# a16z/jolt

Hardware: AMD Instinct MI355X
Metric: prover trace cycles/sec (sha3-shaped synthetic trace, sumcheck + HyperKZG hot path) (higher is better)
Workload: dtype u256 (BN254 Fr / Fq, 8x u32 Montgomery limbs; integer, bit-exact)

## Files before the change

include/jolt_hip.h:

```cpp
#ifndef JOLT_HIP_H
#define JOLT_HIP_H

#include <stddef.h>
#include <stdint.h>

#ifdef __cplusplus
extern "C" {
#endif

#define JOLT_HIP_ABI_VERSION 1

typedef struct { uint64_t l[4]; } jolt_fr_t;
typedef struct { uint64_t l[4]; } jolt_fq_t;
typedef struct { jolt_fq_t x, y, z; } jolt_g1_t;

typedef struct jolt_ctx jolt_ctx;
typedef struct jolt_table jolt_table;
typedef struct jolt_member jolt_member;
typedef struct jolt_srs jolt_srs;

enum {
    JOLT_OK = 0,
    JOLT_ERR_INVALID_ARG = 1,
    JOLT_ERR_NO_DEVICE = 2,
// ... 129 lines not shown

int32_t jolt_msm_g1(jolt_ctx *ctx, const jolt_srs *srs, const jolt_fr_t *scalars, size_t n, jolt_g1_t *out);
int32_t jolt_msm_g1_table(jolt_ctx *ctx, const jolt_srs *srs, const jolt_table *scalars, size_t n, jolt_g1_t *out);
int32_t jolt_msm_g1_table_full_width(jolt_ctx *ctx, const jolt_srs *srs, const jolt_table *scalars, size_t n, jolt_g1_t *out);
typedef struct jolt_msm_pending jolt_msm_pending;
int32_t jolt_msm_g1_tables_begin(jolt_ctx *ctx, const jolt_srs *srs, const jolt_table *const *scalars, const size_t *n, size_t count, jolt_msm_pending **out);
int32_t jolt_msm_g1_tables_finish(jolt_ctx *ctx, jolt_msm_pending *pending, jolt_g1_t *out);

int32_t jolt_hyperkzg_fold(jolt_ctx *ctx, const jolt_table *evals, const jolt_fr_t *point, size_t ell, jolt_table **levels_out);
int32_t jolt_hyperkzg_eval3(jolt_ctx *ctx, jolt_table *const *levels, size_t ell, const jolt_fr_t u[3], jolt_fr_t *v_out);
int32_t jolt_hyperkzg_rlc(jolt_ctx *ctx, jolt_table *const *levels, size_t ell, const jolt_fr_t *q, jolt_table **out);
int32_t jolt_hyperkzg_witness_poly(jolt_ctx *ctx, const jolt_table *f, const jolt_fr_t *u, jolt_table **out);

int32_t jolt_host_fr_mul(const jolt_fr_t *a, const jolt_fr_t *b, jolt_fr_t *out);
int32_t jolt_host_fr_add(const jolt_fr_t *a, const jolt_fr_t *b, jolt_fr_t *out);
int32_t jolt_host_fr_sub(const jolt_fr_t *a, const jolt_fr_t *b, jolt_fr_t *out);
int32_t jolt_host_fr_inv(const jolt_fr_t *a, jolt_fr_t *out);
int32_t jolt_host_fr_from_u64(uint64_t v, jolt_fr_t *out);
int32_t jolt_host_fr_mul_shifted(const jolt_fr_t *a, const jolt_fr_t *c, jolt_fr_t *out);
int32_t jolt_host_eq_evals(const jolt_fr_t *r, size_t n, const jolt_fr_t *scale, jolt_fr_t *out);
int32_t jolt_host_mul_limbs29(int32_t field, const jolt_fr_t *a, const jolt_fr_t *b, jolt_fr_t *out);
int32_t jolt_host_fq_limb_op(int32_t op, const jolt_fr_t *a, const jolt_fr_t *b, const jolt_fr_t *c, const jolt_fr_t *d, jolt_fr_t *out);
int32_t jolt_host_g1_sum_limb_form(const uint64_t *points, const uint8_t *negate, size_t count, jolt_g1_t *out);
int32_t jolt_host_fx_digits(const jolt_fr_t *scalar, uint32_t window_bits, uint32_t *keys_out, uint32_t *n_windows_out, uint32_t *buckets_out);
int32_t jolt_host_fx_segment_capacity(uint64_t n, uint32_t window_bits, uint32_t segment, uint32_t *capacity);
int32_t jolt_host_univariate_from_evals(const jolt_fr_t *evals, size_t n, jolt_fr_t *coeffs_out);
int32_t jolt_host_univariate_evaluate(const jolt_fr_t *coeffs, size_t n, const jolt_fr_t *x, jolt_fr_t *out);
int32_t jolt_host_gruen_poly_from_q(const jolt_fr_t *current_scalar, const jolt_fr_t *point_i, const jolt_fr_t *q_evals, size_t dq,
                                    const jolt_fr_t *s0_plus_s1, jolt_fr_t *coeffs_out);
int32_t jolt_host_gruen_poly_deg_3(const jolt_fr_t *current_scalar, const jolt_fr_t *point_i, const jolt_fr_t *q_constant,
                                   const jolt_fr_t *q_quadratic, const jolt_fr_t *s0_plus_s1, jolt_fr_t *coeffs_out);
int32_t jolt_host_booleanity_address_round(const jolt_fr_t *linear, const jolt_fr_t *squared, size_t n_polys, size_t stride, size_t len,
                                           const jolt_fr_t *weights, const jolt_fr_t *eq_address, jolt_fr_t *evals_out);
int32_t jolt_host_booleanity_address_bind(jolt_fr_t *linear, jolt_fr_t *squared, size_t n_polys, size_t stride, size_t len, jolt_fr_t *eq_address,
                                          const jolt_fr_t *challenge);
int32_t jolt_host_hamming_weights(const jolt_fr_t *gamma, const jolt_fr_t *r_address, const jolt_fr_t *virtualization_points, size_t n_polys, size_t log_k,
                                  jolt_fr_t *out);
int32_t jolt_host_pair_tables_round(const jolt_fr_t *g, const jolt_fr_t *w, size_t n_polys, size_t stride, size_t len, jolt_fr_t *evals_out );
int32_t jolt_host_pair_tables_bind(jolt_fr_t *g, jolt_fr_t *w, size_t n_polys, size_t stride, size_t len, const jolt_fr_t *challenge);
enum { JOLT_TRANSCRIPT_TEST = 0, JOLT_TRANSCRIPT_BLAKE2B_LEGACY = 1, JOLT_TRANSCRIPT_KECCAK_SPONGE = 2, JOLT_TRANSCRIPT_BLAKE2B_SPONGE = 3 };
#define JOLT_TRANSCRIPT_LABEL(kind, label) (((uint64_t)(kind) << 62) | ((uint64_t)(label) & (((uint64_t)1 << 62) - 1)))
typedef struct jolt_host_transcript jolt_host_transcript;
int32_t jolt_host_transcript_create(uint64_t label, jolt_host_transcript **out);
int32_t jolt_host_transcript_create_labelled(int32_t kind, const uint8_t *label, size_t label_len, jolt_host_transcript **out);
int32_t jolt_host_transcript_append_fr(jolt_host_transcript *t, const jolt_fr_t *values, size_t count);
int32_t jolt_host_transcript_append_bytes(jolt_host_transcript *t, const uint8_t *bytes, size_t count);
// ... 297 lines not shown
```

jolt_amd/csrc/fq_limb.hip.h:

```cpp
#pragma once
#include "field.hip.h"

namespace jolt {

struct FqL {
    uint32_t l[9];
};

namespace fql {
constexpr uint32_t P(int k) { return Limbs29<FqParams>::limb(k); }
constexpr uint32_t P2(int k) {
    uint64_t carry = 0, v = 0;
    for (int i = 0; i <= k; ++i) {
        v = 2ull * P(i) + carry;
        carry = v >> 29;
        v &= kMask29;
    }
    return (uint32_t)v;
}
constexpr uint32_t NINV = Limbs29<FqParams>::neg_inv();
constexpr uint32_t PM(int m, int k) {
    uint64_t carry = 0, v = 0;
    for (int i = 0; i <= k; ++i) {
        v = (uint64_t)m * P(i) + carry;
        carry = v >> 29;
        if (i < 8) v &= kMask29;
    }
    return (uint32_t)v;
}
}
#define JOLT_FQL_MP(m) {fql::PM(m, 0), fql::PM(m, 1), fql::PM(m, 2), fql::PM(m, 3), fql::PM(m, 4), fql::PM(m, 5), fql::PM(m, 6), fql::PM(m, 7), fql::PM(m, 8)}
#define JOLT_FQL_P {fql::P(0), fql::P(1), fql::P(2), fql::P(3), fql::P(4), fql::P(5), fql::P(6), fql::P(7), fql::P(8)}
#define JOLT_FQL_2P {fql::P2(0), fql::P2(1), fql::P2(2), fql::P2(3), fql::P2(4), fql::P2(5), fql::P2(6), fql::P2(7), fql::P2(8)}

JOLT_HD FqL fql_from_words(const Fq& a) {
    FqL r;
    to_limbs29<0>(a.l, r.l);
    return r;
}
JOLT_HD FqL fql_zero() {
    FqL r;
#pragma unroll
    for (int k = 0; k < 9; ++k) r.l[k] = 0;
    return r;
}
JOLT_HD bool fql_is_zero(const FqL& a) {
    constexpr uint32_t PL[9] = JOLT_FQL_P;
    uint32_t any = 0, diff = 0;
#pragma unroll
    for (int k = 0; k < 9; ++k) {
        any |= a.l[k];
        diff |= a.l[k] ^ PL[k];
    }
    return any == 0 || diff == 0;
}
JOLT_HD FqL fql_add(const FqL& a, const FqL& b) {
    constexpr uint32_t P2L[9] = JOLT_FQL_2P;
// ... 29 lines not shown
    }
    uint32_t carry = 0;
#pragma unroll
    for (int k = 0; k < 9; ++k) {
        const uint32_t t = d[k] + P2L[k] + carry;
        e[k] = t & kMask29;
        carry = t >> 29;
    }
    FqL r;
#pragma unroll
    for (int k = 0; k < 9; ++k) r.l[k] = borrow ? e[k] : d[k];
    return r;
}
JOLT_HD FqL fql_dbl(const FqL& a) { return fql_add(a, a); }

JOLT_HD FqL fql_mul(const FqL& a, const FqL& b) {
    constexpr uint32_t PL[9] = JOLT_FQL_P;
    uint32_t M[9];
    FqL r;
    uint64_t acc = 0;
#pragma unroll
    for (int k = 0; k < 9; ++k) {
#pragma unroll
        for (int i = 0; i <= k; ++i) acc += (uint64_t)a.l[i] * b.l[k - i];
#pragma unroll
        for (int i = 0; i < k; ++i) acc += (uint64_t)M[i] * PL[k - i];
        M[k] = ((uint32_t)acc * fql::NINV) & kMask29;
        acc += (uint64_t)M[k] * PL[0];
        acc >>= 29;
    }
#pragma unroll
    for (int k = 9; k < 18; ++k) {
#pragma unroll
        for (int i = k - 8; i < 9; ++i) acc += (uint64_t)a.l[i] * b.l[k - i];
#pragma unroll
        for (int i = k - 8; i < 9; ++i) acc += (uint64_t)M[i] * PL[k - i];
        r.l[k - 9] = (uint32_t)acc & kMask29;
        acc >>= 29;
    }
    return r;
}
JOLT_HD FqL fql_mul2(const FqL& a, const FqL& b, const FqL& c, const FqL& d) {
    constexpr uint32_t PL[9] = JOLT_FQL_P;
    uint32_t M[9];
    FqL r;
    uint64_t acc = 0;
#pragma unroll
    for (int k = 0; k < 9; ++k) {
#pragma unroll
        for (int i = 0; i <= k; ++i) {
            acc += (uint64_t)a.l[i] * b.l[k - i];
            acc += (uint64_t)c.l[i] * d.l[k - i];
        }
#pragma unroll
        for (int i = 0; i < k; ++i) acc += (uint64_t)M[i] * PL[k - i];
        M[k] = ((uint32_t)acc * fql::NINV) & kMask29;
        acc += (uint64_t)M[k] * PL[0];
        acc >>= 29;
    }
#pragma unroll
    for (int k = 9; k < 18; ++k) {
#pragma unroll
        for (int i = k - 8; i < 9; ++i) {
            acc += (uint64_t)a.l[i] * b.l[k - i];
            acc += (uint64_t)c.l[i] * d.l[k - i];
        }
#pragma unroll
        for (int i = k - 8; i < 9; ++i) acc += (uint64_t)M[i] * PL[k - i];
        r.l[k - 9] = (uint32_t)acc & kMask29;
        acc >>= 29;
    }
    return r;
}
JOLT_HD FqL fql_sqr(const FqL& a) {
    constexpr uint32_t PL[9] = JOLT_FQL_P;
    uint32_t M[9], a2[9];
#pragma unroll
    for (int k = 0; k < 9; ++k) a2[k] = a.l[k] << 1;
    FqL r;
    uint64_t acc = 0;
#pragma unroll
    for (int k = 0; k < 9; ++k) {
#pragma unroll
        for (int i = 0; 2 * i < k; ++i) acc += (uint64_t)a.l[i] * a2[k - i];
        if (k % 2 == 0) acc += (uint64_t)a.l[k / 2] * a.l[k / 2];
#pragma unroll
        for (int i = 0; i < k; ++i) acc += (uint64_t)M[i] * PL[k - i];
        M[k] = ((uint32_t)acc * fql::NINV) & kMask29;
        acc += (uint64_t)M[k] * PL[0];
        acc >>= 29;
    }
#pragma unroll
    for (int k = 9; k < 18; ++k) {
#pragma unroll
        for (int i = k - 8; 2 * i < k; ++i) acc += (uint64_t)a.l[i] * a2[k - i];
        if (k % 2 == 0) acc += (uint64_t)a.l[k / 2] * a.l[k / 2];
#pragma unroll
        for (int i = k - 8; i < 9; ++i) acc += (uint64_t)M[i] * PL[k - i];
        r.l[k - 9] = (uint32_t)acc & kMask29;
        acc >>= 29;
    }
    return r;
}
JOLT_HD Fq fql_to_std(const FqL& a, const FqL& r256) {
    const FqL v = fql_mul(a, r256);
    Fq out;
#pragma unroll
    for (int j = 0; j < 8; ++j) {
        const int k = (32 * j) / 29, s = 32 * j - 29 * k;
        uint32_t w = v.l[k] >> s;
        w |= v.l[k + 1] << (29 - s);
        if (58 - s < 32 && k + 2 < 9) w |= v.l[k + 2] << (58 - s);
        out.l[j] = w;
    }
    return reduce_once(out, 0u);
}

template <int M, bool WITH_C>
JOLT_HD FqL fql_diff(const FqL& a, const FqL& b, const FqL& c) {
    constexpr uint32_t MP[9] = JOLT_FQL_MP(M);
    FqL r;
    int32_t carry = 0;
#pragma unroll
    for (int k = 0; k < 9; ++k) {
        int32_t t = (int32_t)a.l[k] + (int32_t)MP[k] - (int32_t)b.l[k] + carry;
        if (WITH_C) t -= (int32_t)(c.l[k] << 1);
        r.l[k] = k < 8 ? ((uint32_t)t & kMask29) : (uint32_t)t;
        carry = t >> 29;
    }
    return r;
}
template <int MAX>
JOLT_HD bool fql_is_multiple_of_p(const FqL& a) {
    bool hit = false;
#pragma unroll
    for (int m = 1; m <= MAX; ++m) {
        uint32_t diff = 0;
#pragma unroll
        for (int k = 0; k < 9; ++k) diff |= a.l[k] ^ fql::PM(m, k);
        hit = hit || diff == 0;
    }
    return hit;
}

struct G1XyzzL {
    FqL x, y, zz, zzz;
};
JOLT_HD G1XyzzL g1xl_identity() {
    G1XyzzL r;
// ... 26 lines not shown
        r.zz = one;
        r.zzz = one;
        return r;
    }
    const FqL U2 = fql_mul(qx, p.zz);
    const FqL S2 = fql_mul(qy, p.zzz);
    const FqL P = fql_diff<8, false>(U2, p.x, U2);
    const FqL R = fql_diff<4, false>(S2, p.y, S2);
    const FqL PP = fql_sqr(P);
    const FqL PPP = fql_mul(P, PP);
    const FqL Q = fql_mul(p.x, PP);
    G1XyzzL r;
    r.zz = fql_mul(p.zz, PP);
    if (fql_is_zero(r.zz)) {
        if (fql_is_multiple_of_p<5>(R)) return g1xl_double_affine(qx, qy);
        return g1xl_identity();
    }
    r.x = fql_diff<6, true>(fql_sqr(R), PPP, Q);
    r.y = fql_mul2(R, fql_diff<8, false>(Q, r.x, Q), fql_diff<4, false>(fql_zero(), p.y, Q), PPP);
    r.zzz = fql_mul(p.zzz, PPP);
    return r;
}

}
```

jolt_amd/csrc/host_mirror.hip:

```cpp
#include "host_mirror.hpp"

#include <algorithm>
#include <array>
#include <string>

#include "member.hpp"

using namespace jolt;

namespace jolt_host {

Fr fr_mul_pow_2(Fr a, size_t k) {
    for (size_t i = 0; i < k; ++i) a = add(a, a);
    return a;
}
void fr_to_bytes_le(const Fr& a, uint8_t out[32]) {
    Fr c = from_mont(a);
    for (int i = 0; i < 8; ++i)
        for (int j = 0; j < 4; ++j) out[4 * i + j] = (uint8_t)(c.l[i] >> (8 * j));
}
Fr fr_from_challenge_bytes(const uint8_t* b, size_t n) {
    uint8_t buf[16] = {0};
    std::memcpy(buf, b, n < 16 ? n : 16);
    Fr r = Fr::zero();
// ... 710 lines not shown
    };
    const FqL r256 = fql_from_words(Fq::one());
    FqL r;
    switch (op) {
        case 0: r = fql_mul(load(a), load(b)); break;
        case 1: r = fql_sqr(load(a)); break;
        case 2: r = fql_mul2(load(a), load(b), load(c), load(d)); break;
        case 3: r = fql_mul(fql_diff<8, false>(load(a), load(b), load(a)), load(c)); break;
        case 4: r = fql_mul(fql_diff<6, true>(load(a), load(b), load(c)), load(d)); break;
        default: return JOLT_ERR_INVALID_ARG;
    }
    const Fq res = fql_to_std(r, r256);
    std::memcpy(out, &res, sizeof(res));
    return JOLT_OK;
}
extern "C" int32_t jolt_host_g1_sum_limb_form(const uint64_t* points , const uint8_t* negate, size_t count, jolt_g1_t* out) {
    if ((!points && count) || !out) return JOLT_ERR_INVALID_ARG;
    using namespace jolt;
    Fq thirty_two = Fq::zero();
    thirty_two.l[0] = 32;
    const Fq m32 = to_mont(thirty_two);
    const FqL one = fql_from_words(m32), r256 = fql_from_words(Fq::one());
    G1XyzzL acc = g1xl_identity();
    for (size_t i = 0; i < count; ++i) {
        G1Affine p;
        std::memcpy(&p, points + 8 * i, sizeof(p));
        if (g1_aff_is_inf(p)) continue;
        if (negate && negate[i]) p.y = neg(p.y);
        acc = g1xl_add_mixed(acc, fql_from_words(mul(p.x, m32)), fql_from_words(mul(p.y, m32)), one);
    }
    G1Jac r = g1_identity();
    if (!g1xl_is_identity(acc)) {
        r.x = fql_to_std(fql_mul(acc.x, fql_sqr(acc.zz)), r256);
        r.y = fql_to_std(fql_mul(acc.y, fql_sqr(acc.zzz)), r256);
        r.z = fql_to_std(acc.zzz, r256);
    }
    std::memcpy(out, &r, sizeof(r));
    return JOLT_OK;
}
extern "C" int32_t jolt_host_fr_add(const jolt_fr_t* a, const jolt_fr_t* b, jolt_fr_t* out) {
    if (!a || !b || !out) return JOLT_ERR_INVALID_ARG;
    fr_to_abi(out, add(fr_from_abi(a), fr_from_abi(b)));
    return JOLT_OK;
}
extern "C" int32_t jolt_host_fr_sub(const jolt_fr_t* a, const jolt_fr_t* b, jolt_fr_t* out) {
    if (!a || !b || !out) return JOLT_ERR_INVALID_ARG;
    fr_to_abi(out, sub(fr_from_abi(a), fr_from_abi(b)));
    return JOLT_OK;
}
extern "C" int32_t jolt_host_fr_inv(const jolt_fr_t* a, jolt_fr_t* out) {
    if (!a || !out) return JOLT_ERR_INVALID_ARG;
    Fr v = fr_from_abi(a);
    if (v.is_zero()) return JOLT_ERR_NOT_INVERTIBLE;
    fr_to_abi(out, inv(v));
    return JOLT_OK;
}
extern "C" int32_t jolt_host_fr_from_u64(uint64_t v, jolt_fr_t* out) {
    if (!out) return JOLT_ERR_INVALID_ARG;
    fr_to_abi(out, fr_from_u64(v));
    return JOLT_OK;
// ... 300 lines not shown
```

jolt_amd/csrc/msm_kernels.hip.h:

```cpp
#pragma once
#include "g1.hip.h"
#include "fq_limb.hip.h"
#include "poly_kernels.hip.h"

#ifndef JOLT_BUCKET_WAVES
#define JOLT_BUCKET_WAVES 3
#endif
namespace jolt {
namespace msmk {
namespace {

#ifndef JOLT_BUCKET_XYZZ
#define JOLT_BUCKET_XYZZ 1
#endif
constexpr int kLaneCap = 128;
constexpr int kHeavySeg = 1024;
constexpr int kPeelMax = 16;

__device__ __forceinline__ G1Affine ld_aff(const G1Affine* p) {
    const uint4* q = reinterpret_cast<const uint4*>(p);
    uint4 a = q[0], b = q[1], c = q[2], d = q[3];
    G1Affine r;
    r.x.l[0] = a.x; r.x.l[1] = a.y; r.x.l[2] = a.z; r.x.l[3] = a.w; r.x.l[4] = b.x; r.x.l[5] = b.y; r.x.l[6] = b.z; r.x.l[7] = b.w;
    r.y.l[0] = c.x; r.y.l[1] = c.y; r.y.l[2] = c.z; r.y.l[3] = c.w; r.y.l[4] = d.x; r.y.l[5] = d.y; r.y.l[6] = d.z; r.y.l[7] = d.w;
// ... 197 lines not shown
            if (more) {
                vn = src[kn];
                pn = ld_aff(bases + (vn & 0x7FFFFFFFu));
            }
            if (v >> 31) p.y = neg(p.y);
            acc = JOLT_BUCKET_ADD(acc, p);
            if (!more) break;
            v = vn;
            p = pn;
            k = kn;
        }
        return JOLT_BUCKET_OUT(acc);
    }
#undef JOLT_BUCKET_ADD
#undef JOLT_BUCKET_OUT
}

struct LformConsts {
    Fq one_l;
    Fq r256;
};
__device__ __forceinline__ G1Jac sum_bucket_points_lform(const uint32_t* __restrict__ src, const G1Affine* __restrict__ bases, uint32_t lo, uint32_t hi, uint32_t stride,
                                                         const LformConsts& lc) {
    G1XyzzL acc = g1xl_identity();
    if (lo >= hi) return g1_identity();
    const FqL one = fql_from_words(lc.one_l);
    uint32_t v = src[lo];
    G1Affine p = ld_aff(bases + (v & 0x7FFFFFFFu));
    for (uint32_t k = lo;;) {
        const uint32_t kn = k + stride;
        const bool more = kn < hi;
        uint32_t vn = 0;
        G1Affine pn = p;
        if (more) {
            vn = src[kn];
            pn = ld_aff(bases + (vn & 0x7FFFFFFFu));
        }
        if (!g1_aff_is_inf(p)) {
            if (v >> 31) p.y = neg(p.y);
            acc = g1xl_add_mixed(acc, fql_from_words(p.x), fql_from_words(p.y), one);
        }
        if (!more) break;
        v = vn;
        p = pn;
        k = kn;
    }
    if (g1xl_is_identity(acc)) return g1_identity();
    const FqL r256 = fql_from_words(lc.r256);
    G1Jac out;
    out.x = fql_to_std(fql_mul(acc.x, fql_sqr(acc.zz)), r256);
    out.y = fql_to_std(fql_mul(acc.y, fql_sqr(acc.zzz)), r256);
    out.z = fql_to_std(acc.zzz, r256);
    return out;
}

template <int CH>
__device__ __forceinline__ void stage_indices(uint32_t* __restrict__ col, const uint32_t* __restrict__ src, uint32_t first, uint32_t cnt) {
#pragma unroll 1
    for (int j0 = 0; j0 < CH; j0 += 8) {
        uint32_t t[8];
#pragma unroll
        for (int j = 0; j < 8; ++j) t[j] = first + j0 + j < cnt ? src[first + j0 + j] : 0u;
#pragma unroll
        for (int j = 0; j < 8; ++j) col[(j0 + j) * kBlock] = t[j];
        if (first + j0 + 8 >= cnt) break;
    }
}
template <int CH>
__device__ __forceinline__ G1Jac sum_bucket_points_lform_staged(const uint32_t* __restrict__ src, const G1Affine* __restrict__ bases, uint32_t cnt, const LformConsts& lc,
                                                                uint32_t* __restrict__ col ) {
    if (cnt == 0) return g1_identity();
    G1XyzzL acc = g1xl_identity();
    const FqL one = fql_from_words(lc.one_l);
    stage_indices<CH>(col, src, 0u, cnt);
    uint32_t v = col[0], first = 0;
    G1Affine p = ld_aff(bases + (v & 0x7FFFFFFFu));
    for (uint32_t k = 0;;) {
        const uint32_t kn = k + 1;
        const bool more = kn < cnt;
        uint32_t vn = 0;
        G1Affine pn = p;
        if (more) {
            if (kn - first == (uint32_t)CH) {
                first = kn;
                stage_indices<CH>(col, src, first, cnt);
            }
            vn = col[(kn - first) * kBlock];
            pn = ld_aff(bases + (vn & 0x7FFFFFFFu));
        }
        if (!g1_aff_is_inf(p)) {
            if (v >> 31) p.y = neg(p.y);
            acc = g1xl_add_mixed(acc, fql_from_words(p.x), fql_from_words(p.y), one);
        }
        if (!more) break;
        v = vn;
        p = pn;
        k = kn;
    }
    if (g1xl_is_identity(acc)) return g1_identity();
    const FqL r256 = fql_from_words(lc.r256);
    G1Jac out;
    out.x = fql_to_std(fql_mul(acc.x, fql_sqr(acc.zz)), r256);
    out.y = fql_to_std(fql_mul(acc.y, fql_sqr(acc.zzz)), r256);
    out.z = fql_to_std(acc.zzz, r256);
    return out;
}

template <bool PIPELINED>
__global__ __launch_bounds__(kBlock) __attribute__((amdgpu_waves_per_eu(JOLT_BUCKET_WAVES, JOLT_BUCKET_WAVES))) void k_msm_buckets_light(const uint32_t* __restrict__ hist, const uint32_t* __restrict__ offsets,
                                                             const uint32_t* __restrict__ sorted, const G1Affine* __restrict__ bases, size_t n,
                                                             uint32_t B, int L, uint32_t heavy_threshold, G1Jac* __restrict__ buckets,
                                                             size_t n_windows) {
    uint32_t gt = blockIdx.x * kBlock + threadIdx.x;
    uint32_t b = gt / L + 1, sub = gt % L;
    const size_t wi = (size_t)blockIdx.z * gridDim.y + blockIdx.y;
    if (wi >= n_windows) return;
    const size_t w = n_windows - 1 - wi;
    bool mine = b <= B;
    size_t slot = (size_t)w * (B + 1) + (mine ? b : 0);
    uint32_t cnt = mine ? hist[slot] : 0;
    if (cnt > heavy_threshold) { cnt = 0; mine = false; }
    G1Jac acc = sum_bucket_points<PIPELINED>(sorted + (size_t)w * n + offsets[slot], bases, sub, cnt, (uint32_t)L);
// ... 75 lines not shown
```

jolt_amd/csrc/pcs.hip:

```cpp
#include <algorithm>
#include <cstdlib>
#include <cstring>

#include "grid_hint.hpp"
#include "ints.hpp"
#include "msm_kernels.hip.h"
#include "onehot.hpp"
#include "srs.hpp"
#include "term_map.hip.h"

using namespace jolt;
using namespace jolt::msmk;

int32_t jolt_internal_table_new(jolt_ctx* ctx, size_t len, jolt_table** out);
extern "C" int32_t jolt_grid_commit_onehot_range(jolt_ctx* ctx, const jolt_srs* srs, const jolt_onehot* source, size_t cycle_lo, size_t cycle_hi, jolt_g1_t* out);

namespace {

constexpr int kGridSumBlocks = 512;

template <bool LFORM>
__global__ __launch_bounds__(kBlock) __attribute__((amdgpu_waves_per_eu(JOLT_BUCKET_WAVES, JOLT_BUCKET_WAVES))) void k_grid_onehot_sum(
    const uint8_t* __restrict__ idx, uint32_t wide, size_t grid_cycles, size_t lo, size_t cycles, const G1Affine* __restrict__ bases, G1Jac* __restrict__ partial,
    LformConsts lc, uint32_t shift) {
    const size_t p = blockIdx.y, cls = blockIdx.z;
    const uint8_t* col = hot_col(idx, p * grid_cycles, wide);
    const size_t stride = ((size_t)gridDim.x * kBlock) << shift, folded_cycles = grid_cycles >> shift;
    G1Xyzz acc = g1x_identity();
    G1XyzzL acc_l = g1xl_identity();
    const FqL one = fql_from_words(lc.one_l);
    size_t j = lo + cls + (((size_t)blockIdx.x * kBlock + threadIdx.x) << shift);
    uint32_t a = j < cycles ? hot_load(col, j, wide) : kColdIdx;
    G1Affine pt;
    pt.x = Fq::zero();
    pt.y = Fq::zero();
    if (a != kColdIdx) pt = ld_aff(bases + (size_t)a * folded_cycles + (j >> shift));
    while (j < cycles) {
        const size_t jn = j + stride;
        const uint32_t an = jn < cycles ? hot_load(col, jn, wide) : kColdIdx;
        G1Affine pn;
        pn.x = Fq::zero();
        pn.y = Fq::zero();
        if (an != kColdIdx) pn = ld_aff(bases + (size_t)an * folded_cycles + (jn >> shift));
        if (LFORM) {
            if (!g1_aff_is_inf(pt)) acc_l = g1xl_add_mixed(acc_l, fql_from_words(pt.x), fql_from_words(pt.y), one);
        } else {
            acc = g1x_add_mixed(acc, pt);
        }
        pt = pn;
        j = jn;
    }
    G1Jac mine = g1x_to_jac(acc);
    if (LFORM) {
        mine = g1_identity();
        if (!g1xl_is_identity(acc_l)) {
            const FqL r256 = fql_from_words(lc.r256);
            mine.x = fql_to_std(fql_mul(acc_l.x, fql_sqr(acc_l.zz)), r256);
            mine.y = fql_to_std(fql_mul(acc_l.y, fql_sqr(acc_l.zzz)), r256);
            mine.z = fql_to_std(acc_l.zzz, r256);
        }
    }
    const G1Jac total = wave_sum_g1(mine, 64);
    if ((threadIdx.x & 63) == 0) partial[((cls * gridDim.y + p) * gridDim.x + blockIdx.x) * (kBlock / 64) + (threadIdx.x >> 6)] = total;
}
__global__ __launch_bounds__(64) void k_grid_onehot_fold(const G1Jac* __restrict__ partial, uint32_t count, G1Jac* __restrict__ out, uint32_t n_cols, uint32_t out_cols,
                                                         uint32_t first) {
    const size_t p = blockIdx.x;
    G1Jac acc = g1_identity();
    for (uint32_t k = threadIdx.x; k < count; k += 64) acc = g1_add(acc, partial[p * count + k]);
    acc = wave_sum_g1(acc, 64);
    if (threadIdx.x == 0) out[(p / n_cols) * out_cols + first + (p % n_cols)] = acc;
}
__global__ __launch_bounds__(1024) void k_grid_hint_combine(const G1Jac* __restrict__ points, const Fr* __restrict__ scalars, const uint32_t* __restrict__ offsets,
                                                            G1Jac* __restrict__ out) {
    __shared__ G1Jac wave_total[16];
    const uint32_t lo = offsets[blockIdx.x], hi = offsets[blockIdx.x + 1];
    G1Jac acc = g1_identity();
    for (uint32_t i = lo + threadIdx.x; i < hi; i += blockDim.x) {
// ... 425 lines not shown
```

jolt_amd/ffi.py:

```python
import ctypes as C
import os

import numpy as np

_HERE = os.path.dirname(os.path.abspath(__file__))
LIB_PATH = os.path.join(_HERE, "libjolt_hip.so")

STATUS = {0: "ok", 1: "invalid argument", 2: "no device", 3: "oom", 4: "hip error", 5: "size mismatch", 6: "unsupported",
          7: "not fully bound", 8: "round check failed", 9: "srs too small", 10: "empty point", 11: "not invertible"}
ORDER_LOW_TO_HIGH, ORDER_HIGH_TO_LOW = 0, 1
MEMBER_FLAG_SKIP_ONE = 1
MEMBER_FLAG_BORROW_TABLES = 2


class JoltError(RuntimeError):
    def __init__(self, status, where, detail=""):
        self.status = status
        super().__init__(f"{where}: status {status} ({STATUS.get(status, '?')}) {detail}")


class MemberDesc(C.Structure):
    _fields_ = [("n_tables", C.c_uint32), ("n_terms", C.c_uint32), ("degree", C.c_uint32), ("order", C.c_int32),
                ("term_offsets", C.c_void_p), ("factors", C.c_void_p), ("coeffs", C.c_void_p)]

# ... 1595 lines not shown
        if self.h:
            lib().jolt_read_raf_destroy(self.ctx.h, self.h)
            self.h = None


Context.read_raf = lambda self, lookup_index, table_index, raf_flag, n_tables: ReadRaf(self, lookup_index, table_index, raf_flag, n_tables)


def host_fq_limb_op(op, a, b=None, c=None, d=None):
    o = fr_array(1)
    arg = lambda x: _p(fr(x)) if x is not None else None
    _ck(lib().jolt_host_fq_limb_op(C.c_int32(op), arg(a), arg(b), arg(c), arg(d), _p(o)), "jolt_host_fq_limb_op")
    return o[0]


def host_g1_sum_limb_form(points, negate=None):
    pts = np.ascontiguousarray(points, dtype=np.uint64).reshape(-1, 8)
    neg = np.ascontiguousarray(negate if negate is not None else np.zeros(pts.shape[0]), dtype=np.uint8)
    out = g1_array(1)
    _ck(lib().jolt_host_g1_sum_limb_form(pts.ctypes.data_as(C.c_void_p), neg.ctypes.data_as(C.c_void_p), C.c_size_t(pts.shape[0]), _p(out)), "jolt_host_g1_sum_limb_form")
    return out[0]


def host_fx_digits(scalar, window_bits):
    keys = np.zeros(64, dtype=np.uint32)
    nw, nb = C.c_uint32(), C.c_uint32()
    _ck(lib().jolt_host_fx_digits(_p(fr(scalar)), C.c_uint32(window_bits), keys.ctypes.data_as(C.c_void_p), C.byref(nw), C.byref(nb)), "jolt_host_fx_digits")
    return [(-1 if int(k) >> 31 else 1) * (int(k) & 0x7FFFFFFF) for k in keys[: nw.value]], nb.value


def host_fx_segment_capacity(n, window_bits, segment):
    cap = C.c_uint32()
    _ck(lib().jolt_host_fx_segment_capacity(C.c_uint64(n), C.c_uint32(window_bits), C.c_uint32(segment), C.byref(cap)), "jolt_host_fx_segment_capacity")
    return int(cap.value)


def host_suffix_mle(kind, bits, length):
    out = C.c_uint64()
    _ck(lib().jolt_host_suffix_mle(C.c_uint32(kind), C.c_uint64(bits & (2**64 - 1)), C.c_uint64((bits >> 64) & (2**64 - 1)), C.c_uint32(length), C.byref(out)), "jolt_host_suffix_mle")
    return out.value


def host_small_scalar_dot(values, scalars):
    v = fr(values).reshape(-1, 4)
    sc = np.array([[int(x) & (2**64 - 1), (int(x) >> 64) & (2**64 - 1)] for x in scalars], dtype=np.uint64).reshape(-1, 2)
    o = fr_array(1)
# ... 342 lines not shown
```

rust/jolt-kernels-hip/src/ffi.rs:

```rust
#![allow(non_camel_case_types, clippy::too_many_arguments, clippy::missing_safety_doc)]
use core::ffi::{c_char, c_void};

pub const JOLT_HIP_ABI_VERSION: i32 = 1;

#[repr(C)]
#[derive(Clone, Copy, Debug, Default, PartialEq, Eq)]
pub struct jolt_fr_t {
    pub l: [u64; 4],
}
#[repr(C)]
#[derive(Clone, Copy, Debug, Default, PartialEq, Eq)]
pub struct jolt_fq_t {
    pub l: [u64; 4],
}
#[repr(C)]
#[derive(Clone, Copy, Debug, Default, PartialEq, Eq)]
pub struct jolt_g1_t {
    pub x: jolt_fq_t,
    pub y: jolt_fq_t,
    pub z: jolt_fq_t,
}
#[repr(C)]
pub struct jolt_ctx {
    _private: [u8; 0],
// ... 197 lines not shown
    pub fn jolt_srs_precompute_windows(ctx: *mut jolt_ctx, srs: *mut jolt_srs, window_bits: u32, min_terms: usize) -> i32;
    pub fn jolt_msm_profile_buckets(ctx: *mut jolt_ctx, enable: i32) -> i32;
    pub fn jolt_msm_profile_buckets_last(ctx: *mut jolt_ctx, ms: *mut f32, additions: *mut u64) -> i32;
    pub fn jolt_ctx_measure_mad_peak(ctx: *mut jolt_ctx, target_ms: f32, mads_per_s: *mut f64, timed_ms: *mut f32, launches: *mut u32) -> i32;
    pub fn jolt_msm_g1(ctx: *mut jolt_ctx, srs: *const jolt_srs, scalars: *const jolt_fr_t, n: usize, out: *mut jolt_g1_t) -> i32;
    pub fn jolt_msm_g1_table(ctx: *mut jolt_ctx, srs: *const jolt_srs, scalars: *const jolt_table, n: usize, out: *mut jolt_g1_t) -> i32;
    pub fn jolt_msm_g1_table_full_width(ctx: *mut jolt_ctx, srs: *const jolt_srs, scalars: *const jolt_table, n: usize, out: *mut jolt_g1_t) -> i32;
    pub fn jolt_msm_g1_tables_begin(ctx: *mut jolt_ctx, srs: *const jolt_srs, scalars: *const *const jolt_table, n: *const usize, count: usize, out: *mut *mut jolt_msm_pending) -> i32;
    pub fn jolt_msm_g1_tables_finish(ctx: *mut jolt_ctx, pending: *mut jolt_msm_pending, out: *mut jolt_g1_t) -> i32;
    pub fn jolt_hyperkzg_fold(ctx: *mut jolt_ctx, evals: *const jolt_table, point: *const jolt_fr_t, ell: usize, levels_out: *mut *mut jolt_table) -> i32;
    pub fn jolt_hyperkzg_eval3(ctx: *mut jolt_ctx, levels: *const *mut jolt_table, ell: usize, u: *const jolt_fr_t, v_out: *mut jolt_fr_t) -> i32;
    pub fn jolt_hyperkzg_rlc(ctx: *mut jolt_ctx, levels: *const *mut jolt_table, ell: usize, q: *const jolt_fr_t, out: *mut *mut jolt_table) -> i32;
    pub fn jolt_hyperkzg_witness_poly(ctx: *mut jolt_ctx, f: *const jolt_table, u: *const jolt_fr_t, out: *mut *mut jolt_table) -> i32;
    pub fn jolt_host_fr_mul(a: *const jolt_fr_t, b: *const jolt_fr_t, out: *mut jolt_fr_t) -> i32;
    pub fn jolt_host_fr_add(a: *const jolt_fr_t, b: *const jolt_fr_t, out: *mut jolt_fr_t) -> i32;
    pub fn jolt_host_fr_sub(a: *const jolt_fr_t, b: *const jolt_fr_t, out: *mut jolt_fr_t) -> i32;
    pub fn jolt_host_fr_inv(a: *const jolt_fr_t, out: *mut jolt_fr_t) -> i32;
    pub fn jolt_host_fr_from_u64(v: u64, out: *mut jolt_fr_t) -> i32;
    pub fn jolt_host_fr_mul_shifted(a: *const jolt_fr_t, c: *const jolt_fr_t, out: *mut jolt_fr_t) -> i32;
    pub fn jolt_host_eq_evals(r: *const jolt_fr_t, n: usize, scale: *const jolt_fr_t, out: *mut jolt_fr_t) -> i32;
    pub fn jolt_host_mul_limbs29(field: i32, a: *const jolt_fr_t, b: *const jolt_fr_t, out: *mut jolt_fr_t) -> i32;
    pub fn jolt_host_fq_limb_op(op: i32, a: *const jolt_fr_t, b: *const jolt_fr_t, c: *const jolt_fr_t, d: *const jolt_fr_t, out: *mut jolt_fr_t) -> i32;
    pub fn jolt_host_g1_sum_limb_form(points: *const u64, negate: *const u8, count: usize, out: *mut jolt_g1_t) -> i32;
    pub fn jolt_host_fx_digits(scalar: *const jolt_fr_t, window_bits: u32, keys_out: *mut u32, n_windows_out: *mut u32, buckets_out: *mut u32) -> i32;
    pub fn jolt_host_fx_segment_capacity(n: u64, window_bits: u32, segment: u32, capacity: *mut u32) -> i32;
    pub fn jolt_host_univariate_from_evals(evals: *const jolt_fr_t, n: usize, coeffs_out: *mut jolt_fr_t) -> i32;
    pub fn jolt_host_univariate_evaluate(coeffs: *const jolt_fr_t, n: usize, x: *const jolt_fr_t, out: *mut jolt_fr_t) -> i32;
    pub fn jolt_host_gruen_poly_from_q(current_scalar: *const jolt_fr_t, point_i: *const jolt_fr_t, q_evals: *const jolt_fr_t, dq: usize, s0_plus_s1: *const jolt_fr_t, coeffs_out: *mut jolt_fr_t) -> i32;
    pub fn jolt_host_gruen_poly_deg_3(current_scalar: *const jolt_fr_t, point_i: *const jolt_fr_t, q_constant: *const jolt_fr_t, q_quadratic: *const jolt_fr_t, s0_plus_s1: *const jolt_fr_t, coeffs_out: *mut jolt_fr_t) -> i32;
    pub fn jolt_host_booleanity_address_round(linear: *const jolt_fr_t, squared: *const jolt_fr_t, n_polys: usize, stride: usize, len: usize, weights: *const jolt_fr_t, eq_address: *const jolt_fr_t, evals_out: *mut jolt_fr_t) -> i32;
    pub fn jolt_host_booleanity_address_bind(linear: *mut jolt_fr_t, squared: *mut jolt_fr_t, n_polys: usize, stride: usize, len: usize, eq_address: *mut jolt_fr_t, challenge: *const jolt_fr_t) -> i32;
    pub fn jolt_host_hamming_weights(gamma: *const jolt_fr_t, r_address: *const jolt_fr_t, virtualization_points: *const jolt_fr_t, n_polys: usize, log_k: usize, out: *mut jolt_fr_t) -> i32;
    pub fn jolt_host_pair_tables_round(g: *const jolt_fr_t, w: *const jolt_fr_t, n_polys: usize, stride: usize, len: usize, evals_out: *mut jolt_fr_t) -> i32;
    pub fn jolt_host_pair_tables_bind(g: *mut jolt_fr_t, w: *mut jolt_fr_t, n_polys: usize, stride: usize, len: usize, challenge: *const jolt_fr_t) -> i32;
    pub fn jolt_host_transcript_create(label: u64, out: *mut *mut jolt_host_transcript) -> i32;
    pub fn jolt_host_transcript_create_labelled(kind: i32, label: *const u8, label_len: usize, out: *mut *mut jolt_host_transcript) -> i32;
    pub fn jolt_host_transcript_append_fr(t: *mut jolt_host_transcript, values: *const jolt_fr_t, count: usize) -> i32;
    pub fn jolt_host_transcript_append_bytes(t: *mut jolt_host_transcript, bytes: *const u8, count: usize) -> i32;
    pub fn jolt_host_transcript_append_label(t: *mut jolt_host_transcript, label: *const c_char, with_count: i32, count: u64) -> i32;
    pub fn jolt_host_transcript_append_u64_word(t: *mut jolt_host_transcript, value: u64) -> i32;
    pub fn jolt_host_transcript_append_round_poly(t: *mut jolt_host_transcript, label: *const c_char, coefficients: *const jolt_fr_t, count: usize) -> i32;
    pub fn jolt_host_transcript_challenge(t: *mut jolt_host_transcript, full_width: i32, out: *mut jolt_fr_t) -> i32;
    pub fn jolt_host_transcript_state(t: *const jolt_host_transcript, out32: *mut u8) -> i32;
    pub fn jolt_host_transcript_destroy(t: *mut jolt_host_transcript) -> i32;
    pub fn jolt_host_blake2b(r#in: *const u8, n: usize, outlen: usize, out: *mut u8) -> i32;
    pub fn jolt_host_keccak_f1600(state200: *mut u8) -> i32;
// ... 167 lines not shown
```

Baseline: 11.37 million.

## Split mixed G1 add into branch-free common path with wave-uniform rare fallback

Restructures the limb-form XYZZ mixed addition used in MSM bucket sums and the PCS accumulation. Each loop now seeds the accumulator from the first point, runs a branch-free common addition with a signed-difference trick that folds y-negation into R, and takes the identity/doubling fallback only when a wave-wide vote flags a suspect result, reloading the point from memory in that case. The field mul/sqr inner products are also rewritten to use inline v_mad_u64_u32 accumulate chains with scalar-register constants. The aim is to cut per-add divergence and branch overhead and to shorten the multiply chains. The risk is in correctness of the suspect detection (it checks only limb 0), and in the compiler scheduling the asm chains less well. A host test mirror is added.

```diff
diff --git a/include/jolt_hip.h b/include/jolt_hip.h
--- a/include/jolt_hip.h
+++ b/include/jolt_hip.h
@@ -175,6 +175,7 @@
 int32_t jolt_host_mul_limbs29(int32_t field, const jolt_fr_t *a, const jolt_fr_t *b, jolt_fr_t *out);
 int32_t jolt_host_fq_limb_op(int32_t op, const jolt_fr_t *a, const jolt_fr_t *b, const jolt_fr_t *c, const jolt_fr_t *d, jolt_fr_t *out);
 int32_t jolt_host_g1_sum_limb_form(const uint64_t *points, const uint8_t *negate, size_t count, jolt_g1_t *out);
+int32_t jolt_host_g1xl_add_paths(const uint32_t *acc, const uint32_t *q, int32_t negate, uint32_t *common, uint32_t *full, uint32_t *step, int32_t *suspect, uint32_t *canon);
 int32_t jolt_host_fx_digits(const jolt_fr_t *scalar, uint32_t window_bits, uint32_t *keys_out, uint32_t *n_windows_out, uint32_t *buckets_out);
 int32_t jolt_host_fx_segment_capacity(uint64_t n, uint32_t window_bits, uint32_t segment, uint32_t *capacity);
 int32_t jolt_host_univariate_from_evals(const jolt_fr_t *evals, size_t n, jolt_fr_t *coeffs_out);
diff --git a/jolt_amd/csrc/fq_limb.hip.h b/jolt_amd/csrc/fq_limb.hip.h
--- a/jolt_amd/csrc/fq_limb.hip.h
+++ b/jolt_amd/csrc/fq_limb.hip.h
@@ -1,5 +1,6 @@
 #pragma once
 #include "field.hip.h"
+#include "g1.hip.h"
 
 namespace jolt {
 
@@ -28,11 +29,39 @@
     }
     return (uint32_t)v;
 }
+constexpr uint32_t PM1(int m, int k) {
+    uint64_t carry = 0, v = 0;
+    for (int i = 0; i <= k; ++i) {
+        v = (uint64_t)m * P(i) + 1 + carry;
+        carry = v >> 29;
+        if (i < 8) v &= kMask29;
+    }
+    return (uint32_t)v;
+}
+constexpr uint32_t PM1H(int m, int k) { return (PM1(m, k) >> 1) | (k < 8 ? (PM1(m, k + 1) & 1u) << 28 : 0u); }
+static_assert((PM1(3, 0) & 1u) == 0 && (PM1(11, 0) & 1u) == 0, "m p + ones must be even");
 }
 #define JOLT_FQL_MP(m) {fql::PM(m, 0), fql::PM(m, 1), fql::PM(m, 2), fql::PM(m, 3), fql::PM(m, 4), fql::PM(m, 5), fql::PM(m, 6), fql::PM(m, 7), fql::PM(m, 8)}
 #define JOLT_FQL_P {fql::P(0), fql::P(1), fql::P(2), fql::P(3), fql::P(4), fql::P(5), fql::P(6), fql::P(7), fql::P(8)}
 #define JOLT_FQL_2P {fql::P2(0), fql::P2(1), fql::P2(2), fql::P2(3), fql::P2(4), fql::P2(5), fql::P2(6), fql::P2(7), fql::P2(8)}
 
+#ifndef JOLT_FQL_ONE_CHAIN
+#define JOLT_FQL_ONE_CHAIN 1
+#endif
+JOLT_HD void fql_mac(uint64_t& acc, uint32_t a, uint32_t b) {
+#if defined(__HIP_DEVICE_COMPILE__) && JOLT_FQL_ONE_CHAIN
+    asm("v_mad_u64_u32 %0, vcc, %1, %2, %0" : "+v"(acc) : "v"(a), "v"(b) : "vcc");
+#else
+    acc += (uint64_t)a * b;
+#endif
+}
+JOLT_HD void fql_mac_const(uint64_t& acc, uint32_t a, uint32_t c) {
+#if defined(__HIP_DEVICE_COMPILE__) && JOLT_FQL_ONE_CHAIN
+    asm("v_mad_u64_u32 %0, vcc, %1, %2, %0" : "+v"(acc) : "v"(a), "s"(c) : "vcc");
+#else
+    acc += (uint64_t)a * c;
+#endif
+}
 JOLT_HD FqL fql_from_words(const Fq& a) {
     FqL r;
     to_limbs29<0>(a.l, r.l);
@@ -108,19 +137,19 @@
 #pragma unroll
     for (int k = 0; k < 9; ++k) {
 #pragma unroll
-        for (int i = 0; i <= k; ++i) acc += (uint64_t)a.l[i] * b.l[k - i];
-#pragma unroll
-        for (int i = 0; i < k; ++i) acc += (uint64_t)M[i] * PL[k - i];
+        for (int i = 0; i <= k; ++i) fql_mac(acc, a.l[i], b.l[k - i]);
+#pragma unroll
+        for (int i = 0; i < k; ++i) fql_mac_const(acc, M[i], PL[k - i]);
         M[k] = ((uint32_t)acc * fql::NINV) & kMask29;
-        acc += (uint64_t)M[k] * PL[0];
+        fql_mac_const(acc, M[k], PL[0]);
         acc >>= 29;
     }
 #pragma unroll
     for (int k = 9; k < 18; ++k) {
 #pragma unroll
-        for (int i = k - 8; i < 9; ++i) acc += (uint64_t)a.l[i] * b.l[k - i];
-#pragma unroll
-        for (int i = k - 8; i < 9; ++i) acc += (uint64_t)M[i] * PL[k - i];
+        for (int i = k - 8; i < 9; ++i) fql_mac(acc, a.l[i], b.l[k - i]);
+#pragma unroll
+        for (int i = k - 8; i < 9; ++i) fql_mac_const(acc, M[i], PL[k - i]);
         r.l[k - 9] = (uint32_t)acc & kMask29;
         acc >>= 29;
     }
@@ -135,24 +164,24 @@
     for (int k = 0; k < 9; ++k) {
 #pragma unroll
         for (int i = 0; i <= k; ++i) {
-            acc += (uint64_t)a.l[i] * b.l[k - i];
-            acc += (uint64_t)c.l[i] * d.l[k - i];
+            fql_mac(acc, a.l[i], b.l[k - i]);
+            fql_mac(acc, c.l[i], d.l[k - i]);
         }
 #pragma unroll
-        for (int i = 0; i < k; ++i) acc += (uint64_t)M[i] * PL[k - i];
+        for (int i = 0; i < k; ++i) fql_mac_const(acc, M[i], PL[k - i]);
         M[k] = ((uint32_t)acc * fql::NINV) & kMask29;
-        acc += (uint64_t)M[k] * PL[0];
+        fql_mac_const(acc, M[k], PL[0]);
         acc >>= 29;
     }
 #pragma unroll
     for (int k = 9; k < 18; ++k) {
 #pragma unroll
         for (int i = k - 8; i < 9; ++i) {
-            acc += (uint64_t)a.l[i] * b.l[k - i];
-            acc += (uint64_t)c.l[i] * d.l[k - i];
+            fql_mac(acc, a.l[i], b.l[k - i]);
+            fql_mac(acc, c.l[i], d.l[k - i]);
         }
 #pragma unroll
-        for (int i = k - 8; i < 9; ++i) acc += (uint64_t)M[i] * PL[k - i];
+        for (int i = k - 8; i < 9; ++i) fql_mac_const(acc, M[i], PL[k - i]);
         r.l[k - 9] = (uint32_t)acc & kMask29;
         acc >>= 29;
     }
@@ -168,21 +197,21 @@
 #pragma unroll
     for (int k = 0; k < 9; ++k) {
 #pragma unroll
-        for (int i = 0; 2 * i < k; ++i) acc += (uint64_t)a.l[i] * a2[k - i];
-        if (k % 2 == 0) acc += (uint64_t)a.l[k / 2] * a.l[k / 2];
-#pragma unroll
-        for (int i = 0; i < k; ++i) acc += (uint64_t)M[i] * PL[k - i];
+        for (int i = 0; 2 * i < k; ++i) fql_mac(acc, a.l[i], a2[k - i]);
+        if (k % 2 == 0) fql_mac(acc, a.l[k / 2], a.l[k / 2]);
+#pragma unroll
+        for (int i = 0; i < k; ++i) fql_mac_const(acc, M[i], PL[k - i]);
         M[k] = ((uint32_t)acc * fql::NINV) & kMask29;
-        acc += (uint64_t)M[k] * PL[0];
+        fql_mac_const(acc, M[k], PL[0]);
         acc >>= 29;
     }
 #pragma unroll
     for (int k = 9; k < 18; ++k) {
 #pragma unroll
-        for (int i = k - 8; 2 * i < k; ++i) acc += (uint64_t)a.l[i] * a2[k - i];
-        if (k % 2 == 0) acc += (uint64_t)a.l[k / 2] * a.l[k / 2];
-#pragma unroll
-        for (int i = k - 8; i < 9; ++i) acc += (uint64_t)M[i] * PL[k - i];
+        for (int i = k - 8; 2 * i < k; ++i) fql_mac(acc, a.l[i], a2[k - i]);
+        if (k % 2 == 0) fql_mac(acc, a.l[k / 2], a.l[k / 2]);
+#pragma unroll
+        for (int i = k - 8; i < 9; ++i) fql_mac_const(acc, M[i], PL[k - i]);
         r.l[k - 9] = (uint32_t)acc & kMask29;
         acc >>= 29;
     }
@@ -211,6 +240,19 @@
     for (int k = 0; k < 9; ++k) {
         int32_t t = (int32_t)a.l[k] + (int32_t)MP[k] - (int32_t)b.l[k] + carry;
         if (WITH_C) t -= (int32_t)(c.l[k] << 1);
+        r.l[k] = k < 8 ? ((uint32_t)t & kMask29) : (uint32_t)t;
+        carry = t >> 29;
+    }
+    return r;
+}
+JOLT_HD FqL fql_diff_signed(const FqL& a, const FqL& b, uint32_t m) {
+    constexpr uint32_t BL[9] = {fql::PM1H(3, 0), fql::PM1H(3, 1), fql::PM1H(3, 2), fql::PM1H(3, 3), fql::PM1H(3, 4), fql::PM1H(3, 5), fql::PM1H(3, 6), fql::PM1H(3, 7), fql::PM1H(3, 8)};
+    constexpr uint32_t CL[9] = {fql::PM1H(11, 0), fql::PM1H(11, 1), fql::PM1H(11, 2), fql::PM1H(11, 3), fql::PM1H(11, 4), fql::PM1H(11, 5), fql::PM1H(11, 6), fql::PM1H(11, 7), fql::PM1H(11, 8)};
+    FqL r;
+    int32_t carry = 0;
+#pragma unroll
+    for (int k = 0; k < 9; ++k) {
+        const int32_t t = (((int32_t)a.l[k] - (int32_t)BL[k]) ^ (int32_t)m) + (int32_t)CL[k] - (int32_t)b.l[k] + carry;
         r.l[k] = k < 8 ? ((uint32_t)t & kMask29) : (uint32_t)t;
         carry = t >> 29;
     }
@@ -283,4 +325,67 @@
     return r;
 }
 
-}
+JOLT_HD G1XyzzL g1xl_add_mixed_common(const G1XyzzL& p, const FqL& qx, const FqL& qy, uint32_t neg_mask, bool& suspect) {
+    const FqL U2 = fql_mul(qx, p.zz);
+    const FqL S2 = fql_mul(qy, p.zzz);
+    const FqL P = fql_diff<8, false>(U2, p.x, U2);
+    const FqL R = fql_diff_signed(S2, p.y, neg_mask);
+    const FqL PP = fql_sqr(P);
+    const FqL PPP = fql_mul(P, PP);
+    const FqL Q = fql_mul(p.x, PP);
+    G1XyzzL r;
+    r.zz = fql_mul(p.zz, PP);
+    suspect = r.zz.l[0] == 0u || r.zz.l[0] == fql::P(0);
+    r.x = fql_diff<6, true>(fql_sqr(R), PPP, Q);
+    r.y = fql_mul2(R, fql_diff<8, false>(Q, r.x, Q), fql_diff<4, false>(fql_zero(), p.y, Q), PPP);
+    r.zzz = fql_mul(p.zzz, PPP);
+    return r;
+}
+JOLT_HD FqL fql_signed_y(const FqL& qy, uint32_t neg_mask) {
+    return neg_mask ? fql_diff<1, false>(fql_zero(), qy, qy) : qy;
+}
+JOLT_HD G1XyzzL g1xl_add_mixed_rare(const G1XyzzL& r, bool& ident, const FqL& qx, const FqL& qy, uint32_t neg_mask, const FqL& one) {
+    if (ident) {
+        ident = false;
+        G1XyzzL q;
+        q.x = qx;
+        q.y = fql_signed_y(qy, neg_mask);
+        q.zz = one;
+        q.zzz = one;
+        return q;
+    }
+    if (!fql_is_zero(r.zz)) return r;
+    if (fql_is_multiple_of_p<7>(r.x)) return g1xl_double_affine(qx, fql_signed_y(qy, neg_mask));
+    ident = true;
+    return g1xl_identity();
+}
+JOLT_HD G1XyzzL g1xl_from_affine(const G1Affine& q, uint32_t neg_mask, const FqL& one, bool& ident) {
+    ident = g1_aff_is_inf(q);
+    if (ident) return g1xl_identity();
+    G1XyzzL r;
+    r.x = fql_from_words(q.x);
+    r.y = fql_signed_y(fql_from_words(q.y), neg_mask);
+    r.zz = one;
+    r.zzz = one;
+    return r;
+}
+#if defined(__HIP_DEVICE_COMPILE__)
+#define JOLT_WAVE_ANY(x) __any(x)
+#else
+#define JOLT_WAVE_ANY(x) (x)
+#endif
+JOLT_HD void g1xl_accumulate(G1XyzzL& acc, bool& ident, const G1Affine& q, const G1Affine* __restrict__ src, uint32_t neg_mask, const FqL& one) {
+    bool skip = false;
+    if (JOLT_WAVE_ANY((q.x.l[0] | q.y.l[0]) == 0u)) skip = g1_aff_is_inf(q);
+    if (skip) return;
+    bool suspect;
+    acc = g1xl_add_mixed_common(acc, fql_from_words(q.x), fql_from_words(q.y), neg_mask, suspect);
+    if (JOLT_WAVE_ANY(suspect)) {
+        if (suspect) {
+            const G1Affine again = *src;
+            acc = g1xl_add_mixed_rare(acc, ident, fql_from_words(again.x), fql_from_words(again.y), neg_mask, one);
+        }
+    }
+}
+
+}
diff --git a/jolt_amd/csrc/host_mirror.hip b/jolt_amd/csrc/host_mirror.hip
--- a/jolt_amd/csrc/host_mirror.hip
+++ b/jolt_amd/csrc/host_mirror.hip
@@ -756,20 +756,56 @@
     const Fq m32 = to_mont(thirty_two);
     const FqL one = fql_from_words(m32), r256 = fql_from_words(Fq::one());
     G1XyzzL acc = g1xl_identity();
+    bool ident = true;
     for (size_t i = 0; i < count; ++i) {
         G1Affine p;
         std::memcpy(&p, points + 8 * i, sizeof(p));
-        if (g1_aff_is_inf(p)) continue;
-        if (negate && negate[i]) p.y = neg(p.y);
-        acc = g1xl_add_mixed(acc, fql_from_words(mul(p.x, m32)), fql_from_words(mul(p.y, m32)), one);
-    }
+        p.x = mul(p.x, m32);
+        p.y = mul(p.y, m32);
+        const uint32_t neg_mask = negate && negate[i] ? ~0u : 0u;
+        if (i == 0) acc = g1xl_from_affine(p, neg_mask, one, ident);
+        else g1xl_accumulate(acc, ident, p, &p, neg_mask, one);
+    }
+    if (ident != g1xl_is_identity(acc)) return JOLT_ERR_INVALID_ARG;
     G1Jac r = g1_identity();
-    if (!g1xl_is_identity(acc)) {
+    if (!ident) {
         r.x = fql_to_std(fql_mul(acc.x, fql_sqr(acc.zz)), r256);
         r.y = fql_to_std(fql_mul(acc.y, fql_sqr(acc.zzz)), r256);
         r.z = fql_to_std(acc.zzz, r256);
     }
     std::memcpy(out, &r, sizeof(r));
+    return JOLT_OK;
+}
+extern "C" int32_t jolt_host_g1xl_add_paths(const uint32_t* acc, const uint32_t* q, int32_t negate, uint32_t* common, uint32_t* full, uint32_t* step, int32_t* suspect,
+                                            uint32_t* canon) {
+    if (!acc || !q || !common || !full || !step || !suspect || !canon) return JOLT_ERR_INVALID_ARG;
+    using namespace jolt;
+    Fq thirty_two = Fq::zero();
+    thirty_two.l[0] = 32;
+    const FqL one = fql_from_words(to_mont(thirty_two)), r256 = fql_from_words(Fq::one());
+    G1XyzzL p;
+    FqL qx, qy;
+    std::memcpy(&p, acc, sizeof(p));
+    std::memcpy(&qx, q, sizeof(qx));
+    std::memcpy(&qy, q + 9, sizeof(qy));
+    const uint32_t neg_mask = negate ? ~0u : 0u;
+    bool sus = false;
+    const G1XyzzL c = g1xl_add_mixed_common(p, qx, qy, neg_mask, sus);
+    const G1XyzzL f = g1xl_add_mixed(p, qx, fql_signed_y(qy, neg_mask), one);
+    bool ident = g1xl_is_identity(p);
+    const G1XyzzL s = sus ? g1xl_add_mixed_rare(c, ident, qx, qy, neg_mask, one) : c;
+    std::memcpy(common, &c, sizeof(c));
+    std::memcpy(full, &f, sizeof(f));
+    std::memcpy(step, &s, sizeof(s));
+    *suspect = sus ? 1 : 0;
+    const G1XyzzL* both[2] = {&c, &f};
+    for (int k = 0; k < 2; ++k) {
+        const FqL* co[4] = {&both[k]->x, &both[k]->y, &both[k]->zz, &both[k]->zzz};
+        for (int j = 0; j < 4; ++j) {
+            const Fq v = fql_to_std(*co[j], r256);
+            std::memcpy(canon + (k * 4 + j) * 8, &v, sizeof(v));
+        }
+    }
     return JOLT_OK;
 }
 extern "C" int32_t jolt_host_fr_add(const jolt_fr_t* a, const jolt_fr_t* b, jolt_fr_t* out) {
diff --git a/jolt_amd/csrc/msm_kernels.hip.h b/jolt_amd/csrc/msm_kernels.hip.h
--- a/jolt_amd/csrc/msm_kernels.hip.h
+++ b/jolt_amd/csrc/msm_kernels.hip.h
@@ -243,30 +243,33 @@
 };
 __device__ __forceinline__ G1Jac sum_bucket_points_lform(const uint32_t* __restrict__ src, const G1Affine* __restrict__ bases, uint32_t lo, uint32_t hi, uint32_t stride,
                                                          const LformConsts& lc) {
-    G1XyzzL acc = g1xl_identity();
     if (lo >= hi) return g1_identity();
     const FqL one = fql_from_words(lc.one_l);
     uint32_t v = src[lo];
     G1Affine p = ld_aff(bases + (v & 0x7FFFFFFFu));
-    for (uint32_t k = lo;;) {
-        const uint32_t kn = k + stride;
-        const bool more = kn < hi;
-        uint32_t vn = 0;
-        G1Affine pn = p;
-        if (more) {
-            vn = src[kn];
-            pn = ld_aff(bases + (vn & 0x7FFFFFFFu));
-        }
-        if (!g1_aff_is_inf(p)) {
-            if (v >> 31) p.y = neg(p.y);
-            acc = g1xl_add_mixed(acc, fql_from_words(p.x), fql_from_words(p.y), one);
-        }
-        if (!more) break;
-        v = vn;
-        p = pn;
-        k = kn;
-    }
-    if (g1xl_is_identity(acc)) return g1_identity();
+    bool ident;
+    G1XyzzL acc = g1xl_from_affine(p, (uint32_t)((int32_t)v >> 31), one, ident);
+    if (lo + stride < hi) {
+        uint32_t k = lo + stride;
+        v = src[k];
+        p = ld_aff(bases + (v & 0x7FFFFFFFu));
+        for (;;) {
+            const uint32_t kn = k + stride;
+            const bool more = kn < hi;
+            uint32_t vn = 0;
+            G1Affine pn = p;
+            if (more) {
+                vn = src[kn];
+                pn = ld_aff(bases + (vn & 0x7FFFFFFFu));
+            }
+            g1xl_accumulate(acc, ident, p, bases + (v & 0x7FFFFFFFu), (uint32_t)((int32_t)v >> 31), one);
+            if (!more) break;
+            v = vn;
+            p = pn;
+            k = kn;
+        }
+    }
+    if (ident) return g1_identity();
     const FqL r256 = fql_from_words(lc.r256);
     G1Jac out;
     out.x = fql_to_std(fql_mul(acc.x, fql_sqr(acc.zz)), r256);
@@ -291,34 +294,36 @@
 __device__ __forceinline__ G1Jac sum_bucket_points_lform_staged(const uint32_t* __restrict__ src, const G1Affine* __restrict__ bases, uint32_t cnt, const LformConsts& lc,
                                                                 uint32_t* __restrict__ col ) {
     if (cnt == 0) return g1_identity();
-    G1XyzzL acc = g1xl_identity();
     const FqL one = fql_from_words(lc.one_l);
     stage_indices<CH>(col, src, 0u, cnt);
     uint32_t v = col[0], first = 0;
     G1Affine p = ld_aff(bases + (v & 0x7FFFFFFFu));
-    for (uint32_t k = 0;;) {
-        const uint32_t kn = k + 1;
-        const bool more = kn < cnt;
-        uint32_t vn = 0;
-        G1Affine pn = p;
-        if (more) {
-            if (kn - first == (uint32_t)CH) {
-                first = kn;
-                stage_indices<CH>(col, src, first, cnt);
+    bool ident;
+    G1XyzzL acc = g1xl_from_affine(p, (uint32_t)((int32_t)v >> 31), one, ident);
+    if (cnt > 1) {
+        v = col[kBlock];
+        p = ld_aff(bases + (v & 0x7FFFFFFFu));
+        for (uint32_t k = 1;;) {
+            const uint32_t kn = k + 1;
+            const bool more = kn < cnt;
+            uint32_t vn = 0;
+            G1Affine pn = p;
+            if (more) {
+                if (kn - first == (uint32_t)CH) {
+                    first = kn;
+                    stage_indices<CH>(col, src, first, cnt);
+                }
+                vn = col[(kn - first) * kBlock];
+                pn = ld_aff(bases + (vn & 0x7FFFFFFFu));
             }
-            vn = col[(kn - first) * kBlock];
-            pn = ld_aff(bases + (vn & 0x7FFFFFFFu));
-        }
-        if (!g1_aff_is_inf(p)) {
-            if (v >> 31) p.y = neg(p.y);
-            acc = g1xl_add_mixed(acc, fql_from_words(p.x), fql_from_words(p.y), one);
-        }
-        if (!more) break;
-        v = vn;
-        p = pn;
-        k = kn;
-    }
-    if (g1xl_is_identity(acc)) return g1_identity();
+            g1xl_accumulate(acc, ident, p, bases + (v & 0x7FFFFFFFu), (uint32_t)((int32_t)v >> 31), one);
+            if (!more) break;
+            v = vn;
+            p = pn;
+            k = kn;
+        }
+    }
+    if (ident) return g1_identity();
     const FqL r256 = fql_from_words(lc.r256);
     G1Jac out;
     out.x = fql_to_std(fql_mul(acc.x, fql_sqr(acc.zz)), r256);
diff --git a/jolt_amd/csrc/pcs.hip b/jolt_amd/csrc/pcs.hip
--- a/jolt_amd/csrc/pcs.hip
+++ b/jolt_amd/csrc/pcs.hip
@@ -28,8 +28,18 @@
     const size_t stride = ((size_t)gridDim.x * kBlock) << shift, folded_cycles = grid_cycles >> shift;
     G1Xyzz acc = g1x_identity();
     G1XyzzL acc_l = g1xl_identity();
+    bool ident = true;
     const FqL one = fql_from_words(lc.one_l);
     size_t j = lo + cls + (((size_t)blockIdx.x * kBlock + threadIdx.x) << shift);
+    if (LFORM) {
+        for (; j < cycles; j += stride) {
+            const uint32_t a0 = hot_load(col, j, wide);
+            if (a0 == kColdIdx) continue;
+            acc_l = g1xl_from_affine(ld_aff(bases + (size_t)a0 * folded_cycles + (j >> shift)), 0u, one, ident);
+            j += stride;
+            break;
+        }
+    }
     uint32_t a = j < cycles ? hot_load(col, j, wide) : kColdIdx;
     G1Affine pt;
     pt.x = Fq::zero();
@@ -43,17 +53,18 @@
         pn.y = Fq::zero();
         if (an != kColdIdx) pn = ld_aff(bases + (size_t)an * folded_cycles + (jn >> shift));
         if (LFORM) {
-            if (!g1_aff_is_inf(pt)) acc_l = g1xl_add_mixed(acc_l, fql_from_words(pt.x), fql_from_words(pt.y), one);
+            if (a != kColdIdx) g1xl_accumulate(acc_l, ident, pt, bases + (size_t)a * folded_cycles + (j >> shift), 0u, one);
         } else {
             acc = g1x_add_mixed(acc, pt);
         }
         pt = pn;
+        a = an;
         j = jn;
     }
     G1Jac mine = g1x_to_jac(acc);
     if (LFORM) {
         mine = g1_identity();
-        if (!g1xl_is_identity(acc_l)) {
+        if (!ident) {
             const FqL r256 = fql_from_words(lc.r256);
             mine.x = fql_to_std(fql_mul(acc_l.x, fql_sqr(acc_l.zz)), r256);
             mine.y = fql_to_std(fql_mul(acc_l.y, fql_sqr(acc_l.zzz)), r256);
diff --git a/jolt_amd/ffi.py b/jolt_amd/ffi.py
--- a/jolt_amd/ffi.py
+++ b/jolt_amd/ffi.py
@@ -1641,6 +1641,17 @@
     return out[0]
 
 
+def host_g1xl_add_paths(acc, q, negate=False):
+    a = np.ascontiguousarray(acc, dtype=np.uint32).reshape(36)
+    b = np.ascontiguousarray(q, dtype=np.uint32).reshape(18)
+    common, full, step = (np.zeros((4, 9), dtype=np.uint32) for _ in range(3))
+    canon = np.zeros((2, 4, 8), dtype=np.uint32)
+    sus = C.c_int32()
+    vp = lambda x: x.ctypes.data_as(C.c_void_p)
+    _ck(lib().jolt_host_g1xl_add_paths(vp(a), vp(b), C.c_int32(1 if negate else 0), vp(common), vp(full), vp(step), C.byref(sus), vp(canon)), "jolt_host_g1xl_add_paths")
+    return {"common": common, "full": full, "step": step, "suspect": bool(sus.value), "canon_common": canon[0], "canon_full": canon[1]}
+
+
 def host_fx_digits(scalar, window_bits):
     keys = np.zeros(64, dtype=np.uint32)
     nw, nb = C.c_uint32(), C.c_uint32()
diff --git a/rust/jolt-kernels-hip/src/ffi.rs b/rust/jolt-kernels-hip/src/ffi.rs
--- a/rust/jolt-kernels-hip/src/ffi.rs
+++ b/rust/jolt-kernels-hip/src/ffi.rs
@@ -243,6 +243,7 @@
     pub fn jolt_host_mul_limbs29(field: i32, a: *const jolt_fr_t, b: *const jolt_fr_t, out: *mut jolt_fr_t) -> i32;
     pub fn jolt_host_fq_limb_op(op: i32, a: *const jolt_fr_t, b: *const jolt_fr_t, c: *const jolt_fr_t, d: *const jolt_fr_t, out: *mut jolt_fr_t) -> i32;
     pub fn jolt_host_g1_sum_limb_form(points: *const u64, negate: *const u8, count: usize, out: *mut jolt_g1_t) -> i32;
+    pub fn jolt_host_g1xl_add_paths(acc: *const u32, q: *const u32, negate: i32, common: *mut u32, full: *mut u32, step: *mut u32, suspect: *mut i32, canon: *mut u32) -> i32;
     pub fn jolt_host_fx_digits(scalar: *const jolt_fr_t, window_bits: u32, keys_out: *mut u32, n_windows_out: *mut u32, buckets_out: *mut u32) -> i32;
     pub fn jolt_host_fx_segment_capacity(n: u64, window_bits: u32, segment: u32, capacity: *mut u32) -> i32;
     pub fn jolt_host_univariate_from_evals(evals: *const jolt_fr_t, n: usize, coeffs_out: *mut jolt_fr_t) -> i32;
```

Result: faster. 11.63 million, median of 6 (+2.3%).
